# gmh14/tssplat

Measured on AMD Instinct MI355X. Metric: tetrahedra/sec (energy fwd+bwd), higher is better.
Workload: dtype f32

## Files before the change

### tssplat_amd/_build.py

```python
from __future__ import annotations

import contextlib
import hashlib
import os
import shutil
import subprocess
import sys

_HERE = os.path.dirname(os.path.abspath(__file__))
CSRC = os.path.join(_HERE, "csrc")
LIB = os.path.join(_HERE, "libtssplat_amd.so")
_OBJ = os.path.join(_HERE, "_obj")
ARCH = "gfx950"

SOURCES = ["plan.cpp", "plan_mesh.cpp", "plan_tiling.cpp", "plan_layout.cpp", "plan_planes.cpp", "partition.cpp", "conflict_opt.cpp", "regular_batch.cpp", "capi.cpp", "tile_kernel.hip", "step_kernels.hip", "eval_launch.cpp", "surface.cpp", "surface_capi.cpp", "surface_kernels.hip",
           "raster_capi.cpp", "raster_kernels.hip", "aa_kernels.hip", "grid_capi.cpp", "grid_kernels.hip",
           "mlp_capi.cpp", "mlp_kernels.hip", "texture_capi.cpp", "texture_kernels.hip", "shade_capi.cpp", "shade_kernels.hip",
           "init_capi.cpp", "init_kernels.hip", "merge_capi.cpp", "merge_kernels.hip", "fill_kernels.hip",
           "metrics_capi.cpp", "metrics_kernels.hip", "simplify_capi.cpp", "simplify_kernels.hip", "voxel_capi.cpp", "voxel_kernels.hip"]
HEADERS = ["plan.h", "planner.h", "conflict_opt.h", "kernels.h", "launch_args.h", "regular_batch.h", "surface.h", "raster.h", "grid.h", "mlp.h", "texture.h", "shade.h", "init.h", "merge.h", "metrics.h", "simplify.h", "voxel.h", "det_mean.h", "capi_common.h", os.path.join("..", "..", "include", "tssplat_amd.h")]

HOST_FLAGS = ["-O3", "-std=c++17", "-fPIC", "-Wall", "-Wextra", "-Wno-unused-parameter", "-pthread"]
DEVICE_FLAGS = [f"--offload-arch={ARCH}", "-ffp-contract=fast", "-fno-slp-vectorize", "-mllvm", "-amdgpu-sched-strategy=max-ilp"]
SOURCE_FLAGS = {"raster_kernels.hip": ["-ffp-contract=off"], "aa_kernels.hip": ["-ffp-contract=off"],
                "texture_kernels.hip": ["-ffp-contract=off"], "shade_kernels.hip": ["-ffp-contract=off"],
                "init_kernels.hip": ["-ffp-contract=off"], "merge_kernels.hip": ["-ffp-contract=off"],
                "metrics_kernels.hip": ["-ffp-contract=off"], "simplify_kernels.hip": ["-ffp-contract=off"],
                "voxel_kernels.hip": ["-ffp-contract=off"]}


def _hipcc() -> str:
    for cand in (os.environ.get("HIPCC"), shutil.which("hipcc"), "/opt/rocm/bin/hipcc"):
        if cand and os.path.exists(cand):
            return cand
    raise RuntimeError("hipcc not found: the tssplat_amd extension cannot be built (no CPU fallback exists)")


def _digest() -> str:
    h = hashlib.sha256()
    for name in SOURCES + HEADERS:
        with open(os.path.join(CSRC, name), "rb") as fh:
            h.update(fh.read())
    h.update(" ".join(HOST_FLAGS + DEVICE_FLAGS + [f"{k}:{' '.join(v)}" for k, v in sorted(SOURCE_FLAGS.items())]).encode())
    return h.hexdigest()


def traffic_digest() -> str:
    h = hashlib.sha256()
    planner = sorted(n for n in SOURCES + HEADERS if n.startswith("plan") or n.startswith("partition"))
    for name in ["tile_kernel.hip", "launch_args.h"] + planner:
        with open(os.path.join(CSRC, name), "rb") as fh:
            h.update(fh.read())
    return h.hexdigest()[:16]


def build_variant(name: str, extra_device_flags: list[str]) -> str:
    hipcc = _hipcc()
    out = os.path.join(_HERE, f"libtssplat_amd_{name}.so")
    os.makedirs(_OBJ, exist_ok=True)
    objs = []
    for src in SOURCES:
        obj = os.path.join(_OBJ, f"{os.path.splitext(src)[0]}_{name}.o")
        if src.endswith(".hip"):
            cmd = [hipcc, "-c", os.path.join(CSRC, src), "-o", obj] + HOST_FLAGS + DEVICE_FLAGS + SOURCE_FLAGS.get(src, []) + extra_device_flags
        else:
            cmd = [hipcc] + HOST_FLAGS + ["-x", "c++", "-D__HIP_PLATFORM_AMD__", "-I/opt/rocm/include", "-c",
                                           os.path.join(CSRC, src), "-o", obj] + \
                  [f for f in extra_device_flags if f.startswith("-D")]
        subprocess.check_call(cmd)
        objs.append(obj)
    subprocess.check_call([hipcc, "-shared", "-o", out] + objs + [f"--offload-arch={ARCH}", "-pthread"])
    return out


def _write_atomic(path: str, text: str) -> None:
    tmp = f"{path}.{os.getpid()}.tmp"
    with open(tmp, "w") as fh:
        fh.write(text)
    os.replace(tmp, path)


@contextlib.contextmanager
def _build_lock():
    import fcntl
    with open(os.path.join(_HERE, ".build.lock"), "w") as fh:
        fcntl.flock(fh, fcntl.LOCK_EX)
        try:
            yield
        finally:
            fcntl.flock(fh, fcntl.LOCK_UN)


def build(force: bool = False, verbose: bool = False) -> str:
    stamp = LIB + ".digest"
    if not force and os.path.exists(LIB) and os.path.exists(stamp) and open(stamp).read() == _digest():
        return LIB
    with _build_lock():
        return _build_locked(force, verbose)


def _build_locked(force: bool, verbose: bool) -> str:
    stamp = LIB + ".digest"
    digest = _digest()
    if not force and os.path.exists(LIB) and os.path.exists(stamp) and open(stamp).read() == digest:
        return LIB
    hipcc = _hipcc()
    os.makedirs(_OBJ, exist_ok=True)
# ... 69 lines not shown
```

### tssplat_amd/csrc/eval_launch.cpp

```cpp
#include <vector>

#include "kernels.h"
#include "launch_args.h"

namespace tsamd {

bool lane_layout_supported(int spt, int max_threads) { return tile_kernel_for(spt, max_threads, true, false, false, true) != nullptr; }

hipError_t configure_kernels(int lds_bytes)
{
    static int configured[64] = {};
    int dev = 0;
    if (hipGetDevice(&dev) != hipSuccess || dev < 0 || dev >= 64) dev = 0;
    if (lds_bytes <= configured[dev]) return hipSuccess;
    for (const TileKernelRow &row : kTileKernels)
        for (const void *fn : row.fn) {
            hipFuncAttributes attr;
            hipError_t e = hipFuncGetAttributes(&attr, fn);
            if (e != hipSuccess) return e;
            if (attr.sharedSizeBytes != 0) return hipErrorInvalidDeviceFunction;
            e = hipFuncSetAttribute(fn, hipFuncAttributeMaxDynamicSharedMemorySize, lds_bytes);
            if (e != hipSuccess) return e;
        }
    configured[dev] = lds_bytes;
    return hipSuccess;
}

namespace {

struct LaunchRecipe {
    KernelArgs k;
    FinishArgs f;
    const void *tile_fn = nullptr, *finish_fn = nullptr;
    dim3 tile_grid, tile_block, finish_grid, finish_block;
    size_t tile_lds = 0;
};

void set_coefficients(KernelArgs &k, float c1, float c2)
{
    k.c1 = c1;
    k.c2 = c2;
    k.ratio = c2 / c1;
}

hipError_t make_recipe(const EvalArgs &e, LaunchRecipe &r)
{
    if (e.n_tiles > 0) {
        KernelArgs &k = r.k;
        k.tiles = e.tiles;
        k.blob = e.blob;
        k.gvid = e.gvid;
        k.vdst = e.vdst;
        k.x = e.x;
        k.grad_out = e.grad_out;
        k.grad = e.grad;
        k.stage = e.stage;
        k.partials = e.partials;
        set_coefficients(k, e.c1, e.c2);
        k.coef = e.coef;
        k.order = e.order;
        k.n_tiles = int(e.n_tiles);
        k.tiles_per_xcd = int((e.n_tiles + 7) / 8);
        k.vert_stride = e.vert_stride;
        k.n_planes = e.n_planes;
        k.reg_period = uint32_t(e.regular.period);
        k.reg_mul = e.regular.div_mul;
        k.reg_shift = e.regular.div_shift;
        k.reg_v = e.regular.V;
        k.reg_s = e.regular.S;
        r.tile_fn = tile_kernel_for(e.spt, e.block_threads, e.grad != nullptr, e.weighted, e.rebuild, e.index_nt);
        if (!r.tile_fn) return hipErrorInvalidConfiguration;
        r.tile_block = dim3(unsigned(e.block_threads));
        r.tile_grid = dim3(unsigned(8 * k.tiles_per_xcd));
        r.tile_lds = size_t(e.lds_bytes);
    }
    FinishArgs &f = r.f;
    f.fin_vid = e.fin_vid;
    f.fin_off = e.fin_off;
    f.n_finish = e.grad ? e.n_finish : 0;
    f.stage = e.stage;
    f.grad = e.grad;
    f.grad_out = e.grad_out;
    f.partials = e.partials;
    f.n_tiles = e.n_tiles;
    f.c1 = e.c1;
    f.c2 = e.c2;
    f.coef = e.coef;
    f.energy = e.energy;
    f.terms = e.terms;
    f.energy_copy = nullptr;
    const bool regular = e.regular.period > 0 && e.regular.K > 0 && int64_t(finish_grid(e.regular.K) - 1) * 256 >= e.regular.K;
    f.reg_k = regular ? e.regular.K : 0;
    f.reg_copies = regular ? e.regular.copies : 0;
    f.reg_v = regular ? e.regular.V : 0;
    f.reg_s = regular ? e.regular.S : 0;
    if (f.n_finish > 0) {
        r.finish_fn = step_kernels().finish;
        r.finish_grid = regular ? finish_grid_regular(f.reg_k, f.reg_copies) : dim3(finish_grid(f.n_finish));
        r.finish_block = dim3(256);
    } else if (f.energy) {
        r.finish_fn = step_kernels().energy_reduce;
        r.finish_grid = dim3(1);
        r.finish_block = dim3(1024);
    }
    return hipSuccess;
}

hipError_t add_kernel_node(hipGraph_t graph, hipGraphNode_t prev, hipGraphNode_t *node, hipKernelNodeParams &p, const void *fn, dim3 grid, dim3 block,
                           size_t lds, void **args)
{
    p = hipKernelNodeParams{};
    p.func = const_cast<void *>(fn);
    p.gridDim = grid;
    p.blockDim = block;
    p.sharedMemBytes = unsigned(lds);
    p.kernelParams = args;
    p.extra = nullptr;
    return hipGraphAddKernelNode(node, graph, prev ? &prev : nullptr, prev ? 1 : 0, &p);
}

hipError_t launch_eval_kernels(const EvalArgs &e, hipStream_t stream, hipEvent_t *ev)
{
    LaunchRecipe r;
    hipError_t err = make_recipe(e, r);
    if (err != hipSuccess) return err;
    if (r.tile_fn) {
        void *argv[] = {&r.k};
        err = hipLaunchKernel(r.tile_fn, r.tile_grid, r.tile_block, argv, r.tile_lds, stream);
        if (err != hipSuccess) return err;
    }
    if (ev) {
        err = hipEventRecord(ev[1], stream);
        if (err != hipSuccess) return err;
    }
    if (r.finish_fn) {
        void *argv[] = {&r.f};
        err = hipLaunchKernel(r.finish_fn, r.finish_grid, r.finish_block, argv, 0, stream);
        if (err != hipSuccess) return err;
    }
    return hipSuccess;
}

}

hipError_t launch_eval(const EvalArgs &e, hipStream_t stream, hipEvent_t *ev)
{
    if (ev) {
        hipError_t err = hipEventRecord(ev[0], stream);
        if (err != hipSuccess) return err;
    }
    hipError_t rc = launch_eval_kernels(e, stream, ev);
    if (rc == hipSuccess && ev) rc = hipEventRecord(ev[2], stream);
    return rc;
}

struct EvalGraph {
    LaunchRecipe r;
    hipGraph_t graph = nullptr;
    hipGraphExec_t exec = nullptr;
    hipGraphNode_t tile_node = nullptr, finish_node = nullptr;
    hipKernelNodeParams tile_p, finish_p;
    void *tile_argv[1], *finish_argv[1];
    float *own_grad = nullptr;
};

hipError_t eval_graph_create(const EvalArgs &e, EvalGraph **out)
{
    *out = nullptr;
    EvalGraph *g = new EvalGraph();
    hipError_t err = make_recipe(e, g->r);
    g->own_grad = e.grad;
    auto fail = [&](hipError_t code) {
        eval_graph_destroy(g);
        return code;
    };
    if (err != hipSuccess) return fail(err);
    if ((err = hipGraphCreate(&g->graph, 0)) != hipSuccess) return fail(err);
    const LaunchRecipe &r = g->r;
    if (r.tile_fn) {
        g->tile_argv[0] = &g->r.k;
        if ((err = add_kernel_node(g->graph, nullptr, &g->tile_node, g->tile_p, r.tile_fn, r.tile_grid, r.tile_block, r.tile_lds, g->tile_argv)) != hipSuccess)
            return fail(err);
    }
    if (r.finish_fn) {
        g->finish_argv[0] = &g->r.f;
        if ((err = add_kernel_node(g->graph, g->tile_node, &g->finish_node, g->finish_p, r.finish_fn, r.finish_grid, r.finish_block, 0, g->finish_argv)) !=
            hipSuccess)
            return fail(err);
    }
    if ((err = hipGraphInstantiate(&g->exec, g->graph, nullptr, nullptr, 0)) != hipSuccess) return fail(err);
    *out = g;
    return hipSuccess;
}

hipError_t eval_graph_launch(EvalGraph *g, float c1, float c2, hipStream_t stream, float *energy_copy, float *grad)
{
    hipError_t err;
    const bool coef = g->r.k.c1 != c1 || g->r.k.c2 != c2 || g->r.f.c1 != c1 || g->r.f.c2 != c2;
    if (!grad) grad = g->own_grad;
    if (grad != g->r.f.grad && !g->own_grad) return hipErrorInvalidValue;
    const bool moved = grad != g->r.f.grad;
    if (coef || moved) {
        set_coefficients(g->r.k, c1, c2);
        g->r.f.c1 = c1;
        g->r.f.c2 = c2;
        g->r.k.grad = grad;
        if (g->tile_node && (err = hipGraphExecKernelNodeSetParams(g->exec, g->tile_node, &g->tile_p)) != hipSuccess) return err;
    }
    if (coef || moved || g->r.f.energy_copy != energy_copy) {
        if (energy_copy && (!g->finish_node || !g->r.f.energy)) return hipErrorInvalidValue;
        g->r.f.energy_copy = energy_copy;
        g->r.f.grad = grad;
        if (g->finish_node && (err = hipGraphExecKernelNodeSetParams(g->exec, g->finish_node, &g->finish_p)) != hipSuccess) return err;
    }
    return hipGraphLaunch(g->exec, stream);
}

void eval_graph_destroy(EvalGraph *g)
{
    if (!g) return;
    if (g->exec) (void)hipGraphExecDestroy(g->exec);
    if (g->graph) (void)hipGraphDestroy(g->graph);
    delete g;
}

struct TrainLoopGraph {
    struct Adam {
        const float *grad;
        float *g1, *g2, *p;
        int64_t n;
        float b1, b2, lr, bias1, bias2, limit;
        unsigned int *ws;
    };
    struct Step {
        LaunchRecipe r;
        Adam a;
        hipGraphNode_t tile = nullptr, finish = nullptr, moments = nullptr, apply = nullptr;
        hipKernelNodeParams tile_p, finish_p, moments_p, apply_p;
        void *tile_argv[1], *finish_argv[1], *moments_argv[7], *apply_argv[8];
    };
    std::vector<Step> steps;
    hipGraph_t graph = nullptr;
    hipGraphExec_t exec = nullptr;
};

hipError_t train_loop_create(const EvalArgs &e, float *param, float *g1, float *g2, int64_t n_param, void *ws, int n_iters, TrainLoopGraph **out)
{
    *out = nullptr;
    if (n_iters < 1 || n_iters > 4096 || n_param < 1 || !e.grad || !e.energy) return hipErrorInvalidValue;
    TrainLoopGraph *g = new TrainLoopGraph();
    auto fail = [&](hipError_t code) {
        train_loop_destroy(g);
        return code;
    };
    g->steps.resize(size_t(n_iters));
    const StepKernels sk = step_kernels();
    const dim3 adam_blocks(adam_grid(n_param));
    hipError_t err;
    if ((err = hipGraphCreate(&g->graph, 0)) != hipSuccess) return fail(err);
    hipGraphNode_t prev = nullptr;
    {
        hipMemsetParams m = {};
        m.dst = ws;
        m.elementSize = 4;
        m.width = size_t(2 * n_iters);
        m.height = 1;
        m.value = 0;
        if ((err = hipGraphAddMemsetNode(&prev, g->graph, nullptr, 0, &m)) != hipSuccess) return fail(err);
    }
    for (int k = 0; k < n_iters; ++k) {
        TrainLoopGraph::Step &s = g->steps[size_t(k)];
        EvalArgs ek = e;
        ek.x = param;
        ek.energy = e.energy + k;
        if ((err = make_recipe(ek, s.r)) != hipSuccess) return fail(err);
        const LaunchRecipe &r = s.r;
        auto add = [&](hipGraphNode_t *node, hipKernelNodeParams &p, const void *fn, dim3 grid, dim3 block, size_t lds, void **args) {
            const hipError_t rc = add_kernel_node(g->graph, prev, node, p, fn, grid, block, lds, args);
            if (rc == hipSuccess) prev = *node;
            return rc;
        };
        if (r.tile_fn) {
            s.tile_argv[0] = &s.r.k;
            if ((err = add(&s.tile, s.tile_p, r.tile_fn, r.tile_grid, r.tile_block, r.tile_lds, s.tile_argv)) != hipSuccess) return fail(err);
        }
        if (r.finish_fn) {
            s.finish_argv[0] = &s.r.f;
            if ((err = add(&s.finish, s.finish_p, r.finish_fn, r.finish_grid, r.finish_block, 0, s.finish_argv)) != hipSuccess) return fail(err);
        }
        TrainLoopGraph::Adam &a = s.a;
        a = TrainLoopGraph::Adam{e.grad, g1, g2, param, n_param, 0.9f, 0.999f, 0.f, 1.f, 1.f, -1.f, static_cast<unsigned int *>(ws) + 2 * k};
        void **am = s.moments_argv, **aa = s.apply_argv;
        am[0] = &a.grad, am[1] = &a.g1, am[2] = &a.g2, am[3] = &a.n, am[4] = &a.b1, am[5] = &a.b2, am[6] = &a.ws;
        aa[0] = &a.p, aa[1] = &a.g1, aa[2] = &a.n, aa[3] = &a.lr, aa[4] = &a.bias1, aa[5] = &a.bias2, aa[6] = &a.limit, aa[7] = &a.ws;
        if ((err = add(&s.moments, s.moments_p, sk.adam_moments, adam_blocks, dim3(256), 0, am)) != hipSuccess) return fail(err);
        if ((err = add(&s.apply, s.apply_p, sk.adam_apply, adam_blocks, dim3(256), 0, aa)) != hipSuccess) return fail(err);
    }
    if ((err = hipGraphInstantiate(&g->exec, g->graph, nullptr, nullptr, 0)) != hipSuccess) return fail(err);
    *out = g;
    return hipSuccess;
}

hipError_t train_loop_launch(TrainLoopGraph *g, const TrainLoopStep *steps, float lr, float b1, float b2, hipStream_t stream)
{
    hipError_t err;
    for (size_t k = 0; k < g->steps.size(); ++k) {
        TrainLoopGraph::Step &st = g->steps[k];
        LaunchRecipe &r = st.r;
        const TrainLoopStep &s = steps[k];
        if (r.k.c1 != s.c1 || r.k.c2 != s.c2 || r.k.order != s.order || r.f.c1 != s.c1 || r.f.c2 != s.c2) {
            set_coefficients(r.k, s.c1, s.c2);
            r.f.c1 = s.c1;
            r.f.c2 = s.c2;
            r.k.order = s.order;
            if (st.tile && (err = hipGraphExecKernelNodeSetParams(g->exec, st.tile, &st.tile_p)) != hipSuccess) return err;
            if (st.finish && (err = hipGraphExecKernelNodeSetParams(g->exec, st.finish, &st.finish_p)) != hipSuccess) return err;
        }
        TrainLoopGraph::Adam &a = st.a;
        if (a.b1 != b1 || a.b2 != b2) {
            a.b1 = b1;
            a.b2 = b2;
            if ((err = hipGraphExecKernelNodeSetParams(g->exec, st.moments, &st.moments_p)) != hipSuccess) return err;
        }
        if (a.lr != lr || a.bias1 != s.bias1 || a.bias2 != s.bias2 || a.limit != s.limit) {
            a.lr = lr;
            a.bias1 = s.bias1;
            a.bias2 = s.bias2;
            a.limit = s.limit;
            if ((err = hipGraphExecKernelNodeSetParams(g->exec, st.apply, &st.apply_p)) != hipSuccess) return err;
        }
    }
    return hipGraphLaunch(g->exec, stream);
}

void train_loop_destroy(TrainLoopGraph *g)
{
    if (!g) return;
    if (g->exec) (void)hipGraphExecDestroy(g->exec);
    if (g->graph) (void)hipGraphDestroy(g->graph);
    delete g;
}

}
```

### tssplat_amd/csrc/launch_args.h

```cpp
#pragma once

#include <hip/hip_runtime_api.h>

#include <cstdint>

#include "plan.h"

namespace tsamd {

struct KernelArgs {
    const TileDesc *tiles;
    const uint8_t *blob;
    const int32_t *gvid;
    const int32_t *vdst;
    const float *x;
    const float *grad_out;
    float *grad;
    float *stage;
    double *partials;
    float c1, c2;
    float ratio;
    const float *coef;
    int order;
    int n_tiles;
    int tiles_per_xcd;
    int vert_stride;
    int n_planes;
    uint32_t reg_period, reg_mul, reg_shift;
    int reg_v, reg_s;
};

struct FinishArgs {
    const int32_t *fin_vid, *fin_off;
    int64_t n_finish;
    const float *stage;
    float *grad;
    const float *grad_out;
    const double *partials;
    int64_t n_tiles;
    float c1, c2;
    const float *coef;
    float *energy;
    double *terms;
    float *energy_copy;
    int64_t reg_k;
    int reg_copies, reg_v, reg_s;
};

struct TileKernelRow {
    int spt, cap;
    bool weighted, rebuild;
    bool index_nt;
    const void *fn[2];
};
extern const TileKernelRow kTileKernels[9];
const void *tile_kernel_for(int spt, int block_threads, bool grad, bool weighted, bool rebuild, bool index_nt);

struct StepKernels {
    const void *finish, *energy_reduce;
    const void *adam_moments, *adam_apply;
};
StepKernels step_kernels();
unsigned finish_grid(int64_t n_finish);
dim3 finish_grid_regular(int64_t per_copy, int copies);
unsigned adam_grid(int64_t n);

}
```

### tssplat_amd/csrc/tile_kernel.hip

```cpp
#include <hip/hip_runtime.h>

#include "launch_args.h"

namespace tsamd {
namespace {

constexpr int kWave = 64;

#define SLOT_FENCE() __builtin_amdgcn_sched_barrier(0)
#define STAGE_PRIORITY(n) __builtin_amdgcn_s_setprio(n)
#define UNDEF(x) asm volatile("" : "=v"(x))
typedef uint32_t v4u __attribute__((ext_vector_type(4)));
typedef uint32_t v2u __attribute__((ext_vector_type(2)));

__device__ __forceinline__ float det3(const float *F)
{
    return -F[2] * F[4] * F[6] + F[1] * F[5] * F[6] + F[2] * F[3] * F[7] - F[0] * F[5] * F[7] - F[1] * F[3] * F[8] +
           F[0] * F[4] * F[8];
}

__device__ __forceinline__ void cof3(const float *F, float *C)
{
    C[0] = F[4] * F[8] - F[5] * F[7];
    C[1] = F[5] * F[6] - F[3] * F[8];
    C[2] = F[3] * F[7] - F[4] * F[6];
    C[3] = F[2] * F[7] - F[1] * F[8];
    C[4] = F[0] * F[8] - F[2] * F[6];
    C[5] = F[1] * F[6] - F[0] * F[7];
    C[6] = F[1] * F[5] - F[2] * F[4];
    C[7] = F[2] * F[3] - F[0] * F[5];
    C[8] = F[0] * F[4] - F[1] * F[3];
}

#define GLOBAL_AS __attribute__((address_space(1)))
template <class T>
__device__ __forceinline__ GLOBAL_AS T *as_global(T *p)
{
    return (GLOBAL_AS T *)p;
}

typedef float v2f __attribute__((ext_vector_type(2)));
typedef float v4f __attribute__((ext_vector_type(4)));

#define LDS_AS __attribute__((address_space(3)))
template <class T>
__device__ __forceinline__ LDS_AS T *lds_at(uint32_t byte_addr)
{
    return (LDS_AS T *)(uintptr_t)byte_addr;
}

template <class VF>
__device__ __forceinline__ void slot_F(uint32_t xs, uint32_t o0, uint32_t o1, uint32_t o2, uint32_t o3,
                                       const VF *dm, int p, float *F)
{
    const v4u r0 = *lds_at<const v4u>(xs + o0), r1 = *lds_at<const v4u>(xs + o1),
              r2 = *lds_at<const v4u>(xs + o2), r3 = *lds_at<const v4u>(xs + o3);
    asm volatile("" : : "v"(r0), "v"(r1), "v"(r2), "v"(r3));
    const float3 x0 = make_float3(__uint_as_float(r0.x), __uint_as_float(r0.y), __uint_as_float(r0.z));
    const float3 x1 = make_float3(__uint_as_float(r1.x), __uint_as_float(r1.y), __uint_as_float(r1.z));
    const float3 x2 = make_float3(__uint_as_float(r2.x), __uint_as_float(r2.y), __uint_as_float(r2.z));
    const float3 x3 = make_float3(__uint_as_float(r3.x), __uint_as_float(r3.y), __uint_as_float(r3.z));
    const float Ds[9] = {x1.x - x0.x, x2.x - x0.x, x3.x - x0.x, x1.y - x0.y, x2.y - x0.y,
                         x3.y - x0.y, x1.z - x0.z, x2.z - x0.z, x3.z - x0.z};
#pragma unroll
    for (int i = 0; i < 3; ++i)
#pragma unroll
        for (int j = 0; j < 3; ++j)
            F[3 * i + j] = Ds[3 * i + 0] * dm[j][p] + Ds[3 * i + 1] * dm[3 + j][p] + Ds[3 * i + 2] * dm[6 + j][p];
}

template <class VF>
__device__ __forceinline__ void rebuild_dminv(uint32_t rs, uint32_t o0, uint32_t o1, uint32_t o2, uint32_t o3,
                                              VF *dm, int p)
{
    const v4u r0 = *lds_at<const v4u>(rs + o0), r1 = *lds_at<const v4u>(rs + o1),
              r2 = *lds_at<const v4u>(rs + o2), r3 = *lds_at<const v4u>(rs + o3);
    asm volatile("" : : "v"(r0), "v"(r1), "v"(r2), "v"(r3));
    const float x0 = __uint_as_float(r0.x), y0 = __uint_as_float(r0.y), z0 = __uint_as_float(r0.z);
    const float D[9] = {__uint_as_float(r1.x) - x0, __uint_as_float(r2.x) - x0, __uint_as_float(r3.x) - x0,
                        __uint_as_float(r1.y) - y0, __uint_as_float(r2.y) - y0, __uint_as_float(r3.y) - y0,
                        __uint_as_float(r1.z) - z0, __uint_as_float(r2.z) - z0, __uint_as_float(r3.z) - z0};
    float C[9];
    cof3(D, C);
    const float det = D[0] * C[0] + D[1] * C[1] + D[2] * C[2];
    float r = __builtin_amdgcn_rcpf(det);
    r = __builtin_fmaf(__builtin_fmaf(-det, r, 1.f), r, r);
    r = det != 0.f ? r : 0.f;
#pragma unroll
    for (int i = 0; i < 3; ++i)
#pragma unroll
        for (int k = 0; k < 3; ++k) dm[3 * i + k][p] = C[3 * k + i] * r;
}

struct Mat9 {
    v2f p01, p23, p45, p67;
    float p8;
};

__device__ __forceinline__ uint32_t own_token_addr(uint32_t idx) { return 48u * idx + ((idx >> 1) & 12u); }

__device__ __forceinline__ Mat9 load_slot(uint32_t t)
{
    const uint32_t s = t & ~15u;
    const v4f a = *lds_at<const v4f>(s + 16), b = *lds_at<const v4f>(s + 32);
    Mat9 m;
    m.p01 = a.xy; m.p23 = a.zw; m.p45 = b.xy; m.p67 = b.zw;
    m.p8 = *lds_at<const float>(t);
    return m;
}

__device__ __forceinline__ void store_slot(uint32_t t, const float *m)
{
    const uint32_t s = t & ~15u;
    *lds_at<v4f>(s + 16) = v4f{m[0], m[1], m[2], m[3]};
    *lds_at<v4f>(s + 32) = v4f{m[4], m[5], m[6], m[7]};
    *lds_at<float>(t) = m[8];
}

__device__ __forceinline__ void sub9(Mat9 &acc, const Mat9 &g)
{
    acc.p01 -= g.p01; acc.p23 -= g.p23; acc.p45 -= g.p45; acc.p67 -= g.p67;
    acc.p8 -= g.p8;
}

__device__ __forceinline__ Mat9 mat9_of(const float *m)
{
    Mat9 r;
    r.p01 = v2f{m[0], m[1]}; r.p23 = v2f{m[2], m[3]}; r.p45 = v2f{m[4], m[5]}; r.p67 = v2f{m[6], m[7]};
    r.p8 = m[8];
    return r;
}

__device__ __forceinline__ Mat9 laplace_gather(Mat9 acc, const uint32_t *nb)
{
    Mat9 g0 = load_slot(nb[0]);
    acc.p01 *= 4.f; acc.p23 *= 4.f; acc.p45 *= 4.f; acc.p67 *= 4.f;
    acc.p8 *= 4.f;
    Mat9 g1 = load_slot(nb[1]);
    sub9(acc, g0);
    g0 = load_slot(nb[2]);
    sub9(acc, g1);
    g1 = load_slot(nb[3]);
    sub9(acc, g0);
    sub9(acc, g1);
    return acc;
}

__device__ __forceinline__ Mat9 operator_gather(const Mat9 &own, float dg, const float *w, const uint32_t *nb)
{
    Mat9 acc;
    acc.p01 = own.p01 * dg; acc.p23 = own.p23 * dg; acc.p45 = own.p45 * dg; acc.p67 = own.p67 * dg;
    acc.p8 = own.p8 * dg;
#pragma unroll
    for (int k = 0; k < 4; ++k) {
        const Mat9 g = load_slot(nb[k]);
        acc.p01 += g.p01 * w[k]; acc.p23 += g.p23 * w[k]; acc.p45 += g.p45 * w[k]; acc.p67 += g.p67 * w[k];
        acc.p8 += g.p8 * w[k];
    }
    return acc;
}

template <int CTRL>
__device__ __forceinline__ double dpp_f64(double v)
{
    const v2u w = __builtin_bit_cast(v2u, v);
    const v2u r = {uint32_t(__builtin_amdgcn_update_dpp(0, int(w.x), CTRL, 0xf, 0xf, false)),
                   uint32_t(__builtin_amdgcn_update_dpp(0, int(w.y), CTRL, 0xf, 0xf, false))};
    return __builtin_bit_cast(double, r);
}
__device__ __forceinline__ double row_sum_f64(double v)
{
    v += dpp_f64<0xB1>(v);
    v += dpp_f64<0x4E>(v);
    v += dpp_f64<0x124>(v);
    v += dpp_f64<0x128>(v);
    return v;
}

__device__ __forceinline__ float wave_sum(float v)
{
#define TSAMD_DPP(x, ctrl) __builtin_bit_cast(float, __builtin_amdgcn_update_dpp(0, __builtin_bit_cast(int, x), ctrl, 0xf, 0xf, false))
    v += TSAMD_DPP(v, 0xB1);
    v += TSAMD_DPP(v, 0x4E);
    v += TSAMD_DPP(v, 0x124);
    v += TSAMD_DPP(v, 0x128);
#undef TSAMD_DPP
    const int b = __builtin_bit_cast(int, v);
    const float r0 = __builtin_bit_cast(float, __builtin_amdgcn_readlane(b, 0)), r1 = __builtin_bit_cast(float, __builtin_amdgcn_readlane(b, 16)),
                r2 = __builtin_bit_cast(float, __builtin_amdgcn_readlane(b, 32)), r3 = __builtin_bit_cast(float, __builtin_amdgcn_readlane(b, 48));
    return (r0 + r1) + (r2 + r3);
}

constexpr uint32_t kXS = kRowTabBytes;
constexpr uint32_t kZeroEntry = 4u * 66u;

__device__ __forceinline__ uint32_t pos_lo(uint32_t w) { return (w & kVertMask) << 4; }
__device__ __forceinline__ uint32_t pos_hi(uint32_t w) { return ((w >> 16) & kVertMask) << 4; }

template <bool WITH_GRAD, bool WEIGHTED, bool REBUILD, int SPT, bool INDEX_NT>
__device__ __forceinline__ void tile_body(const KernelArgs &a, const int tile, int32_t gv0, const uint32_t reg_vert_off, const int reg_cv, const int reg_cs)
{
    extern __shared__ __attribute__((aligned(16))) unsigned char smem[];
    typedef uint32_t VU __attribute__((ext_vector_type(SPT)));
    typedef float VF __attribute__((ext_vector_type(SPT)));
    static_assert(!(REBUILD && WEIGHTED), "rebuild_dminv is built for the built-in operator");
    constexpr int kKeepF = SPT, kKeepH = WEIGHTED ? 0 : SPT;
    const TileDesc td = a.tiles[tile];
    const int tid = threadIdx.x, nthr = blockDim.x;
    typedef const __attribute__((address_space(4))) float *ConstF;
    const float k_c1 = a.coef ? ((ConstF)(uintptr_t)a.coef)[0] : a.c1, k_c2 = a.coef ? ((ConstF)(uintptr_t)a.coef)[1] : a.c2;
    const float grad_out_scale = WITH_GRAD && a.grad_out ? *(ConstF)(uintptr_t)a.grad_out : 1.f;
    const auto g_blob = as_global(a.blob);
    const auto g_gvid = as_global(a.gvid);
    const auto g_vdst = as_global(a.vdst);
    const auto g_x = as_global(a.x);
    const auto g_grad = as_global(a.grad);
    const auto g_stage = as_global(a.stage);
    const auto g_partials = as_global(a.partials);
    const uint32_t VP = uint32_t(td.n_verts + 3) & ~3u;
    const uint32_t RS = kXS + 16u * VP;
    const uint32_t RB = uint32_t(td.rec_base);
    LDS_AS double *red = lds_at<double>(RB - 256u);
    const int nq = td.s_pad / SPT;
    const bool active = tid < nq;
    const GLOBAL_AS uint32_t *pl = reinterpret_cast<const GLOBAL_AS uint32_t *>(g_blob + td.blob_off);
    const int lt = active ? tid : 0;
    typedef VU PlaneU __attribute__((aligned(SPT == 3 ? 4 : 4 * SPT)));
    typedef VF PlaneF __attribute__((aligned(SPT == 3 ? 4 : 4 * SPT)));
    auto plane_f = [&](int q) -> VF { return __builtin_nontemporal_load(reinterpret_cast<const GLOBAL_AS PlaneF *>(pl + q * td.s_pad + SPT * lt)); };
    constexpr bool kPaired = planes_paired(SPT);
    typedef uint32_t VU2 __attribute__((ext_vector_type(2 * SPT)));
    typedef float VF2 __attribute__((ext_vector_type(2 * SPT)));
    const GLOBAL_AS uint32_t *pli = reinterpret_cast<const GLOBAL_AS uint32_t *>(g_blob + uint64_t(td.stage_off));
#define INDEX_LOAD(p) (INDEX_NT ? __builtin_nontemporal_load(p) : *(p))
    auto pair_u = [&](int q, VU &lo, VU &hi) {
        if (kPaired) {
            const VU2 t = INDEX_LOAD(reinterpret_cast<const GLOBAL_AS VU2 *>(pli + q * td.s_pad + 2 * SPT * lt));
#pragma unroll
            for (int p = 0; p < SPT; ++p) lo[p] = t[p], hi[p] = t[SPT + p];
        } else {
            lo = INDEX_LOAD(reinterpret_cast<const GLOBAL_AS PlaneU *>(pli + q * td.s_pad + SPT * lt));
            hi = INDEX_LOAD(reinterpret_cast<const GLOBAL_AS PlaneU *>(pli + (q + 1) * td.s_pad + SPT * lt));
        }
    };
    auto pair_f = [&](int q, VF &lo, VF &hi) {
        if (kPaired) {
            const VF2 t = __builtin_nontemporal_load(reinterpret_cast<const GLOBAL_AS VF2 *>(pl + q * td.s_pad + 2 * SPT * lt));
#pragma unroll
            for (int p = 0; p < SPT; ++p) lo[p] = t[p], hi[p] = t[SPT + p];
        } else {
            lo = plane_f(q), hi = plane_f(q + 1);
        }
    };
    asm volatile("" : "+v"(gv0));
    float px, py, pz;
    {
        const size_t gv = size_t(gv0 + reg_cv) * 3;
        px = g_x[gv], py = g_x[gv + 1], pz = g_x[gv + 2];
    }
    __builtin_amdgcn_sched_barrier(0);
    VU q_lv01, q_lv23, q_nb01, q_nb23;
    pair_u(0, q_lv01, q_lv23);
    VF dm[9];
    const int kBasePlanes = REBUILD ? kPlanesRebuild : (WEIGHTED ? a.n_planes : kPlanes);
    const GLOBAL_AS uint16_t *g_rowtab = reinterpret_cast<const GLOBAL_AS uint16_t *>(pli + size_t(kBasePlanes) * td.s_pad);
    const GLOBAL_AS v4f *g_rest = reinterpret_cast<const GLOBAL_AS v4f *>(reinterpret_cast<const GLOBAL_AS uint16_t *>(pl + size_t(kBasePlanes) * td.s_pad) + kRowTabEntries);
    v4f rest0 = v4f{0.f, 0.f, 0.f, 0.f};
    if (REBUILD) rest0 = g_rest[tid < td.n_verts ? tid : 0];
    __builtin_amdgcn_sched_barrier(0);
    if (!REBUILD) {
#pragma unroll
        for (int c = 0; c < 8; c += 2) pair_f(4 + c, dm[c], dm[c + 1]);
        dm[8] = plane_f(12);
    }
    __builtin_amdgcn_sched_barrier(0);
    if (tid < td.n_verts) {
        *lds_at<v4f>(kXS + 16u * uint32_t(tid)) = v4f{px, py, pz, 0.f};
        if (REBUILD) *lds_at<v4f>(RS + 16u * uint32_t(tid)) = rest0;
    }
    for (int v = tid + nthr; v < td.n_verts; v += nthr) {
        const size_t gv = size_t(g_gvid[td.vert_off + v]) * 3;
        *lds_at<v4f>(kXS + 16u * uint32_t(v)) = v4f{g_x[gv], g_x[gv + 1], g_x[gv + 2], 0.f};
        if (REBUILD) *lds_at<v4f>(RS + 16u * uint32_t(v)) = g_rest[v];
    }
    __syncthreads();
    pair_u(2, q_nb01, q_nb23);
    VF wd, wk[4];
    if (WEIGHTED) {
        wd = plane_f(13);
        pair_f(14, wk[0], wk[1]);
        pair_f(16, wk[2], wk[3]);
    }
    uint32_t row0 = 0;
    if (WITH_GRAD) row0 = INDEX_LOAD(&g_rowtab[tid < 65 ? tid : 64]);
    __builtin_amdgcn_sched_barrier(0);

    const float ratio = a.coef ? k_c2 / k_c1 : a.ratio;
    const bool factored = k_c1 != 0.f && __builtin_fabsf(ratio) <= 0x1p+40f;
    const float s_pen = factored ? ratio : k_c2, out_scale = factored ? k_c1 : 1.f, q_scale = factored ? 1.f : k_c1;
    uint32_t t_own_reg[SPT];
#pragma unroll
    for (int p = 0; p < SPT; ++p) t_own_reg[p] = RB + own_token_addr(uint32_t(p * nq + tid));
    auto t_own_at = [&](int p) -> uint32_t {
        if (!WEIGHTED) return t_own_reg[p];
        uint32_t t = uint32_t(tid);
        asm volatile("" : "+v"(t));
        return RB + own_token_addr(uint32_t(p * nq) + t);
    };
#define t_own(p) t_own_at(p)
    auto is_owned = [&](int p) { return p * nq + tid < td.n_owned; };

    STAGE_PRIORITY(0);
    float scal[SPT];
#pragma unroll
    for (int p = 0; p < SPT; ++p) scal[p] = 0.f;
    float e_b = 0.f, e_s = 0.f;
    float Fk[kKeepF > 0 ? kKeepF : 1][9];
#pragma unroll
    for (int p = 0; p < kKeepF; ++p)
#pragma unroll
        for (int c = 0; c < 9; ++c) UNDEF(Fk[p][c]);
    if (active) {
#pragma unroll
        for (int p = 0; p < SPT; ++p) {
            const uint32_t w0 = q_lv01[p], w1 = q_lv23[p];
            if (REBUILD) rebuild_dminv(RS, pos_lo(w0), pos_hi(w0), pos_lo(w1), pos_hi(w1), dm, p);
            float F[9];
            slot_F(kXS, pos_lo(w0), pos_hi(w0), pos_lo(w1), pos_hi(w1), dm, p, F);
            if (p < kKeepF) {
#pragma unroll
                for (int c = 0; c < 9; ++c) Fk[p][c] = F[c];
            }
            if (is_owned(p)) {
                const float J = det3(F);
                const float Jm = fmaxf(-J, 0.f);
                float pen = 0.f, dpen = 0.f;
                if (a.order == 2) {
                    pen = Jm * Jm;
                    dpen = -2.f * Jm;
                } else if (a.order == 4) {
                    pen = Jm * Jm * Jm * Jm;
                    dpen = -4.f * Jm * Jm * Jm;
                }
// ... 132 lines not shown
            for (int p = 0; p < SPT; ++p)
#pragma unroll
                for (int c = 0; c < 9; ++c) UNDEF(D[p][c]);
        }
        uint32_t fdst[SPT][4];
#pragma unroll
        for (int p = 0; p < SPT; ++p) {
            const uint32_t w0 = q_lv01[p], w1 = q_lv23[p];
            const uint32_t r0 = *lds_at<const uint32_t>((w0 >> 8) & 0xfcu), r1 = *lds_at<const uint32_t>((w0 >> 24) & 0xfcu),
                           r2 = *lds_at<const uint32_t>((w1 >> 8) & 0xfcu), r3 = *lds_at<const uint32_t>((w1 >> 24) & 0xfcu);
            fdst[p][0] = (w0 & kVertMask) * 12u + r0;
            fdst[p][1] = ((w0 >> 16) & kVertMask) * 12u + r1;
            fdst[p][2] = (w1 & kVertMask) * 12u + r2;
            fdst[p][3] = ((w1 >> 16) & kVertMask) * 12u + r3;
        }
        int vb0 = wave;
        if (wave & 4) {
            const int g4 = wave & ~3, top = g4 + 3 < nw - 1 ? g4 + 3 : nw - 1;
            vb0 = g4 + (top - wave);
        }
        int32_t dst_row = 0;
        if (64 * vb0 + lane < td.n_verts) dst_row = INDEX_LOAD(&g_vdst[reg_vert_off + uint32_t(64 * vb0 + lane)]);
        __syncthreads();
        STAGE_PRIORITY(3);
        if (active) {
#pragma unroll
            for (int p = 0; p < SPT; ++p) {
                if (p * nq + tid < td.n_slots) {
                    const float *d = D[p];
                    LDS_AS float *f0 = lds_at<float>(fdst[p][0]), *f1 = lds_at<float>(fdst[p][1]), *f2 = lds_at<float>(fdst[p][2]),
                                 *f3 = lds_at<float>(fdst[p][3]);
                    f0[0] = (-d[0] - d[3]) - d[6], f0[1] = (-d[1] - d[4]) - d[7], f0[2] = (-d[2] - d[5]) - d[8];
                    f1[0] = d[0], f1[1] = d[1], f1[2] = d[2];
                    f2[0] = d[3], f2[1] = d[4], f2[2] = d[5];
                    f3[0] = d[6], f3[1] = d[7], f3[2] = d[8];
                }
            }
        }
        __syncthreads();

        const float gscale = grad_out_scale * out_scale;
        const uint32_t tab = *lds_at<const uint32_t>(4u * uint32_t(lane));
        const uint32_t wid = *lds_at<const uint32_t>(4u * uint32_t(lane) + 4u) - tab;
        auto vertex_sums = [&](int vb, int32_t row, int cv, int cs) {
            const int v = 64 * vb + lane;
            const uint32_t v12 = 12u * uint32_t(v);
            const int rows = __builtin_popcountll(__builtin_amdgcn_ballot_w64(wid > 768u * uint32_t(vb)));
            float gx = 0.f, gy = 0.f, gz = 0.f;
            for (int r = 0; r < rows; r += 4) {
                const LDS_AS float *f[4];
#pragma unroll
                for (int u = 0; u < 4; ++u) {
                    const uint32_t base = uint32_t(__builtin_amdgcn_readlane(int(tab), r + u)), w = uint32_t(__builtin_amdgcn_readlane(int(wid), r + u));
                    f[u] = lds_at<const float>(v12 < w ? base + v12 : kZeroEntry);
                }
#pragma unroll
                for (int u = 0; u < 4; ++u) {
                    gx += f[u][0];
                    gy += f[u][1];
                    gz += f[u][2];
                }
            }
            if (v < td.n_verts) {
                const bool excl = row >= 0;
                GLOBAL_AS float *dst = (excl ? g_grad : g_stage) + size_t(excl ? row + cv : ~row + cs) * 3;
                const float sc = excl ? gscale : out_scale;
                dst[0] = gx * sc;
                dst[1] = gy * sc;
                dst[2] = gz * sc;
            }
        };
        if (64 * vb0 < td.n_verts) vertex_sums(vb0, dst_row, reg_cv, reg_cs);
        if (64 * nw < td.n_verts) {
            for (int vb = vb0 + nw; 64 * vb < td.n_verts; vb += nw)
                vertex_sums(vb, 64 * vb + lane < td.n_verts ? g_vdst[td.vert_off + 64 * vb + lane] : 0, 0, 0);
        }
        sum_waves();
    }
#undef t_own
#undef INDEX_LOAD
}

template <bool WITH_GRAD, bool WEIGHTED, bool REBUILD, int SPT, bool INDEX_NT>
__device__ __forceinline__ void tile_entry(const KernelArgs &a)
{
    const int xcd = blockIdx.x & 7, jb = blockIdx.x >> 3;
    const int tile_end = (xcd + 1) * a.tiles_per_xcd < a.n_tiles ? (xcd + 1) * a.tiles_per_xcd : a.n_tiles;
    const int tile = xcd * a.tiles_per_xcd + jb;
    if (jb >= a.tiles_per_xcd || tile >= tile_end) return;
    const uint32_t reg_c = uint32_t((uint64_t(uint32_t(tile)) * a.reg_mul) >> a.reg_shift);
    const uint32_t reg_r = uint32_t(tile) - reg_c * a.reg_period;
    const uint32_t reg_vert_off = reg_r * uint32_t(a.vert_stride);
    const GLOBAL_AS int32_t *gv_ptr = &as_global(a.gvid)[size_t(reg_r) * size_t(a.vert_stride) + size_t(int(threadIdx.x) < a.vert_stride ? threadIdx.x : 0)];
    const int32_t gv0 = INDEX_NT ? __builtin_nontemporal_load(gv_ptr) : *gv_ptr;
    __builtin_amdgcn_sched_barrier(0);
    tile_body<WITH_GRAD, WEIGHTED, REBUILD, SPT, INDEX_NT>(a, tile, gv0, reg_vert_off, int(reg_c) * a.reg_v, int(reg_c) * a.reg_s);
}

template <bool WITH_GRAD, int BLOCK, int WPE, bool WEIGHTED = false, bool REBUILD = false, int SPT = kSlotsPerLane>
__global__ __launch_bounds__(BLOCK, WPE) void tile_energy_kernel(const KernelArgs a)
{
    tile_entry<WITH_GRAD, WEIGHTED, REBUILD, SPT, true>(a);
}

template <bool WITH_GRAD, int BLOCK, int WPE, bool WEIGHTED = false, bool REBUILD = false>
__global__ __launch_bounds__(BLOCK, WPE) void tile_shared_index_kernel(const KernelArgs a)
{
    tile_entry<WITH_GRAD, WEIGHTED, REBUILD, kSlotsPerLane, false>(a);
}

}

#define TSAMD_FN(...) {reinterpret_cast<const void *>(&tile_energy_kernel<false, __VA_ARGS__>), reinterpret_cast<const void *>(&tile_energy_kernel<true, __VA_ARGS__>)}
#define TSAMD_FN_SHARED(...) {reinterpret_cast<const void *>(&tile_shared_index_kernel<false, __VA_ARGS__>), reinterpret_cast<const void *>(&tile_shared_index_kernel<true, __VA_ARGS__>)}
const TileKernelRow kTileKernels[9] = {
    {2, 768, true, false, false, TSAMD_FN_SHARED(768, 6, true, false)},
    {2, 768, false, true, false, TSAMD_FN_SHARED(768, 6, false, true)},
    {2, 768, false, false, false, TSAMD_FN_SHARED(768, 6, false, false)},
    {2, 768, true, false, true, TSAMD_FN(768, 6, true, false, 2)},
    {2, 768, false, true, true, TSAMD_FN(768, 6, false, true, 2)},
    {2, 768, false, false, true, TSAMD_FN(768, 6, false, false, 2)},
    {3, 512, false, false, true, TSAMD_FN(512, 4, false, false, 3)},
    {4, 768, false, false, true, TSAMD_FN(768, 3, false, false, 4)},
    {3, 1024, false, false, true, TSAMD_FN(1024, 4, false, false, 3)},
};
#undef TSAMD_FN
#undef TSAMD_FN_SHARED

const void *tile_kernel_for(int spt, int block_threads, bool grad, bool weighted, bool rebuild, bool index_nt)
{
    rebuild = rebuild && !weighted;
    for (const TileKernelRow &row : kTileKernels)
        if (row.spt == spt && block_threads <= row.cap && row.weighted == weighted && row.rebuild == rebuild && (row.index_nt || !index_nt))
            return row.fn[grad];
    return nullptr;
}

}
```

Baseline: 65.71 billion.

## Preload tile kernel head arguments into SGPRs and prefetch the tile descriptor early

Splits the tile kernel's argument struct into 14 dwords of scalar head parameters (tile count, division constants, stride, and the gvid/tiles/x/blob pointers), passed as separate kernel arguments and preloaded into SGPRs with the kernarg-preload compiler flag. The descriptor is loaded in the entry function as three quads, and the vertex position load moves ahead of the coefficient loads. The coefficient and grad_out loads become unconditional scalar loads that fall back to a dummy address. The aim is to shorten each block's startup latency from kernarg memory loads. In exchange it adds a fragile ABI coupling through the static_assert on the 14-dword window, and touches every launch path.

```diff
diff --git a/tssplat_amd/_build.py b/tssplat_amd/_build.py
--- a/tssplat_amd/_build.py
+++ b/tssplat_amd/_build.py
@@ -22,7 +22,8 @@
 
 HOST_FLAGS = ["-O3", "-std=c++17", "-fPIC", "-Wall", "-Wextra", "-Wno-unused-parameter", "-pthread"]
 DEVICE_FLAGS = [f"--offload-arch={ARCH}", "-ffp-contract=fast", "-fno-slp-vectorize", "-mllvm", "-amdgpu-sched-strategy=max-ilp"]
-SOURCE_FLAGS = {"raster_kernels.hip": ["-ffp-contract=off"], "aa_kernels.hip": ["-ffp-contract=off"],
+SOURCE_FLAGS = {"tile_kernel.hip": ["-mllvm", "-amdgpu-kernarg-preload-count=16"],
+                "raster_kernels.hip": ["-ffp-contract=off"], "aa_kernels.hip": ["-ffp-contract=off"],
                 "texture_kernels.hip": ["-ffp-contract=off"], "shade_kernels.hip": ["-ffp-contract=off"],
                 "init_kernels.hip": ["-ffp-contract=off"], "merge_kernels.hip": ["-ffp-contract=off"],
                 "metrics_kernels.hip": ["-ffp-contract=off"], "simplify_kernels.hip": ["-ffp-contract=off"],
diff --git a/tssplat_amd/csrc/eval_launch.cpp b/tssplat_amd/csrc/eval_launch.cpp
--- a/tssplat_amd/csrc/eval_launch.cpp
+++ b/tssplat_amd/csrc/eval_launch.cpp
@@ -29,6 +29,7 @@
 namespace {
 
 struct LaunchRecipe {
+    TileHeadArgs h;
     KernelArgs k;
     FinishArgs f;
     const void *tile_fn = nullptr, *finish_fn = nullptr;
@@ -46,12 +47,13 @@
 hipError_t make_recipe(const EvalArgs &e, LaunchRecipe &r)
 {
     if (e.n_tiles > 0) {
+        TileHeadArgs &h = r.h;
         KernelArgs &k = r.k;
-        k.tiles = e.tiles;
-        k.blob = e.blob;
-        k.gvid = e.gvid;
+        h.tiles = e.tiles;
+        h.blob = e.blob;
+        h.gvid = e.gvid;
         k.vdst = e.vdst;
-        k.x = e.x;
+        h.x = e.x;
         k.grad_out = e.grad_out;
         k.grad = e.grad;
         k.stage = e.stage;
@@ -59,19 +61,18 @@
         set_coefficients(k, e.c1, e.c2);
         k.coef = e.coef;
         k.order = e.order;
-        k.n_tiles = int(e.n_tiles);
-        k.tiles_per_xcd = int((e.n_tiles + 7) / 8);
-        k.vert_stride = e.vert_stride;
+        h.n_tiles = int(e.n_tiles);
+        h.vert_stride = e.vert_stride;
         k.n_planes = e.n_planes;
-        k.reg_period = uint32_t(e.regular.period);
-        k.reg_mul = e.regular.div_mul;
-        k.reg_shift = e.regular.div_shift;
-        k.reg_v = e.regular.V;
+        h.reg_period = uint32_t(e.regular.period);
+        h.reg_mul = e.regular.div_mul;
+        h.reg_shift = e.regular.div_shift;
+        h.reg_v = e.regular.V;
         k.reg_s = e.regular.S;
         r.tile_fn = tile_kernel_for(e.spt, e.block_threads, e.grad != nullptr, e.weighted, e.rebuild, e.index_nt);
         if (!r.tile_fn) return hipErrorInvalidConfiguration;
         r.tile_block = dim3(unsigned(e.block_threads));
-        r.tile_grid = dim3(unsigned(8 * k.tiles_per_xcd));
+        r.tile_grid = dim3(unsigned(8 * tiles_per_xcd(h.n_tiles)));
         r.tile_lds = size_t(e.lds_bytes);
     }
     FinishArgs &f = r.f;
@@ -125,7 +126,8 @@
     hipError_t err = make_recipe(e, r);
     if (err != hipSuccess) return err;
     if (r.tile_fn) {
-        void *argv[] = {&r.k};
+        void *argv[kTileKernelParams];
+        tile_kernel_params(r.h, r.k, argv);
         err = hipLaunchKernel(r.tile_fn, r.tile_grid, r.tile_block, argv, r.tile_lds, stream);
         if (err != hipSuccess) return err;
     }
@@ -160,7 +162,7 @@
     hipGraphExec_t exec = nullptr;
     hipGraphNode_t tile_node = nullptr, finish_node = nullptr;
     hipKernelNodeParams tile_p, finish_p;
-    void *tile_argv[1], *finish_argv[1];
+    void *tile_argv[kTileKernelParams], *finish_argv[1];
     float *own_grad = nullptr;
 };
 
@@ -178,7 +180,7 @@
     if ((err = hipGraphCreate(&g->graph, 0)) != hipSuccess) return fail(err);
     const LaunchRecipe &r = g->r;
     if (r.tile_fn) {
-        g->tile_argv[0] = &g->r.k;
+        tile_kernel_params(g->r.h, g->r.k, g->tile_argv);
         if ((err = add_kernel_node(g->graph, nullptr, &g->tile_node, g->tile_p, r.tile_fn, r.tile_grid, r.tile_block, r.tile_lds, g->tile_argv)) != hipSuccess)
             return fail(err);
     }
@@ -237,7 +239,7 @@
         Adam a;
         hipGraphNode_t tile = nullptr, finish = nullptr, moments = nullptr, apply = nullptr;
         hipKernelNodeParams tile_p, finish_p, moments_p, apply_p;
-        void *tile_argv[1], *finish_argv[1], *moments_argv[7], *apply_argv[8];
+        void *tile_argv[kTileKernelParams], *finish_argv[1], *moments_argv[7], *apply_argv[8];
     };
     std::vector<Step> steps;
     hipGraph_t graph = nullptr;
@@ -281,7 +283,7 @@
             return rc;
         };
         if (r.tile_fn) {
-            s.tile_argv[0] = &s.r.k;
+            tile_kernel_params(s.r.h, s.r.k, s.tile_argv);
             if ((err = add(&s.tile, s.tile_p, r.tile_fn, r.tile_grid, r.tile_block, r.tile_lds, s.tile_argv)) != hipSuccess) return fail(err);
         }
         if (r.finish_fn) {
diff --git a/tssplat_amd/csrc/launch_args.h b/tssplat_amd/csrc/launch_args.h
--- a/tssplat_amd/csrc/launch_args.h
+++ b/tssplat_amd/csrc/launch_args.h
@@ -8,12 +8,34 @@
 
 namespace tsamd {
 
+#define TSAMD_TILE_HEAD_FIELDS(X)                                                                                                              \
+    X(int, n_tiles)                                                                                                                            \
+        \
+             \
+                                                                         \
+    X(uint32_t, reg_mul)                                                                                                                       \
+    X(uint32_t, reg_shift)                                                                                                                     \
+    X(uint32_t, reg_period)                                                                                                                    \
+    X(int, reg_v)                                                                                                                              \
+    X(int, vert_stride)         \
+    X(const int32_t *, gvid)                                                                                                                 \
+    X(const TileDesc *, tiles)                                                                                                                 \
+    X(const float *, x)                                                                                                                        \
+    X(const uint8_t *, blob)
+
+struct TileHeadArgs {
+#define TSAMD_X(type, name) type name;
+    TSAMD_TILE_HEAD_FIELDS(TSAMD_X)
+#undef TSAMD_X
+};
+#define TSAMD_X(type, name) +1
+constexpr int kTileHeadParams = 0 TSAMD_TILE_HEAD_FIELDS(TSAMD_X);
+#undef TSAMD_X
+constexpr int kTileKernelParams = kTileHeadParams + 1;
+static_assert(sizeof(TileHeadArgs) == 14 * 4, "the head arguments are sized for the 14-dword preload window, without padding");
+
 struct KernelArgs {
-    const TileDesc *tiles;
-    const uint8_t *blob;
-    const int32_t *gvid;
     const int32_t *vdst;
-    const float *x;
     const float *grad_out;
     float *grad;
     float *stage;
@@ -22,13 +44,20 @@
     float ratio;
     const float *coef;
     int order;
-    int n_tiles;
-    int tiles_per_xcd;
-    int vert_stride;
     int n_planes;
-    uint32_t reg_period, reg_mul, reg_shift;
-    int reg_v, reg_s;
+    int reg_s;
 };
+
+constexpr int tiles_per_xcd(int n_tiles) { return (n_tiles + 7) >> 3; }
+
+inline void tile_kernel_params(TileHeadArgs &h, KernelArgs &k, void *(&argv)[kTileKernelParams])
+{
+    int n = 0;
+#define TSAMD_X(type, name) argv[n++] = &h.name;
+    TSAMD_TILE_HEAD_FIELDS(TSAMD_X)
+#undef TSAMD_X
+    argv[n] = &k;
+}
 
 struct FinishArgs {
     const int32_t *fin_vid, *fin_off;
diff --git a/tssplat_amd/csrc/tile_kernel.hip b/tssplat_amd/csrc/tile_kernel.hip
--- a/tssplat_amd/csrc/tile_kernel.hip
+++ b/tssplat_amd/csrc/tile_kernel.hip
@@ -41,6 +41,11 @@
 
 typedef float v2f __attribute__((ext_vector_type(2)));
 typedef float v4f __attribute__((ext_vector_type(4)));
+
+struct TileDescWords {
+    v4u q0, q1, q2;
+};
+static_assert(sizeof(TileDescWords) == sizeof(TileDesc), "a tile descriptor is three quads");
 
 #define LDS_AS __attribute__((address_space(3)))
 template <class T>
@@ -198,22 +203,35 @@
 __device__ __forceinline__ uint32_t pos_hi(uint32_t w) { return ((w >> 16) & kVertMask) << 4; }
 
 template <bool WITH_GRAD, bool WEIGHTED, bool REBUILD, int SPT, bool INDEX_NT>
-__device__ __forceinline__ void tile_body(const KernelArgs &a, const int tile, int32_t gv0, const uint32_t reg_vert_off, const int reg_cv, const int reg_cs)
+__device__ __forceinline__ void tile_body(const TileHeadArgs &h, const KernelArgs &a, const int tile, int32_t gv0, TileDescWords tdw, const uint32_t reg_vert_off, const int reg_cv,
+                                          const int reg_cs)
 {
     extern __shared__ __attribute__((aligned(16))) unsigned char smem[];
     typedef uint32_t VU __attribute__((ext_vector_type(SPT)));
     typedef float VF __attribute__((ext_vector_type(SPT)));
     static_assert(!(REBUILD && WEIGHTED), "rebuild_dminv is built for the built-in operator");
     constexpr int kKeepF = SPT, kKeepH = WEIGHTED ? 0 : SPT;
-    const TileDesc td = a.tiles[tile];
     const int tid = threadIdx.x, nthr = blockDim.x;
+    const auto g_blob = as_global(h.blob);
+    const auto g_gvid = as_global(h.gvid);
+    const auto g_vdst = as_global(a.vdst);
+    const auto g_x = as_global(h.x);
+    asm volatile("" : "+v"(gv0));
+    float px, py, pz;
+    {
+        const size_t gv = size_t(gv0 + reg_cv) * 3;
+        px = g_x[gv], py = g_x[gv + 1], pz = g_x[gv + 2];
+    }
+    __builtin_amdgcn_sched_barrier(0);
+    asm volatile("" : "+s"(tdw.q0), "+s"(tdw.q1), "+s"(tdw.q2));
+    const TileDesc td = __builtin_bit_cast(TileDesc, tdw);
     typedef const __attribute__((address_space(4))) float *ConstF;
-    const float k_c1 = a.coef ? ((ConstF)(uintptr_t)a.coef)[0] : a.c1, k_c2 = a.coef ? ((ConstF)(uintptr_t)a.coef)[1] : a.c2;
-    const float grad_out_scale = WITH_GRAD && a.grad_out ? *(ConstF)(uintptr_t)a.grad_out : 1.f;
-    const auto g_blob = as_global(a.blob);
-    const auto g_gvid = as_global(a.gvid);
-    const auto g_vdst = as_global(a.vdst);
-    const auto g_x = as_global(a.x);
+    typedef v2f CoefPair __attribute__((aligned(4)));
+    typedef const __attribute__((address_space(4))) CoefPair *ConstF2;
+    const v2f dev_coef = *(ConstF2)(uintptr_t)(a.coef ? (const void *)a.coef : (const void *)h.tiles);
+    const float dev_grad_out = *(ConstF)(uintptr_t)(WITH_GRAD && a.grad_out ? (const void *)a.grad_out : (const void *)h.tiles);
+    const float k_c1 = a.coef ? dev_coef.x : a.c1, k_c2 = a.coef ? dev_coef.y : a.c2;
+    const float grad_out_scale = WITH_GRAD && a.grad_out ? dev_grad_out : 1.f;
     const auto g_grad = as_global(a.grad);
     const auto g_stage = as_global(a.stage);
     const auto g_partials = as_global(a.partials);
@@ -252,13 +270,6 @@
             lo = plane_f(q), hi = plane_f(q + 1);
         }
     };
-    asm volatile("" : "+v"(gv0));
-    float px, py, pz;
-    {
-        const size_t gv = size_t(gv0 + reg_cv) * 3;
-        px = g_x[gv], py = g_x[gv + 1], pz = g_x[gv + 2];
-    }
-    __builtin_amdgcn_sched_barrier(0);
     VU q_lv01, q_lv23, q_nb01, q_nb23;
     pair_u(0, q_lv01, q_lv23);
     VF dm[9];
@@ -557,32 +568,40 @@
 }
 
 template <bool WITH_GRAD, bool WEIGHTED, bool REBUILD, int SPT, bool INDEX_NT>
-__device__ __forceinline__ void tile_entry(const KernelArgs &a)
+__device__ __forceinline__ void tile_entry(const TileHeadArgs &h, const KernelArgs &a)
 {
     const int xcd = blockIdx.x & 7, jb = blockIdx.x >> 3;
-    const int tile_end = (xcd + 1) * a.tiles_per_xcd < a.n_tiles ? (xcd + 1) * a.tiles_per_xcd : a.n_tiles;
-    const int tile = xcd * a.tiles_per_xcd + jb;
-    if (jb >= a.tiles_per_xcd || tile >= tile_end) return;
-    const uint32_t reg_c = uint32_t((uint64_t(uint32_t(tile)) * a.reg_mul) >> a.reg_shift);
-    const uint32_t reg_r = uint32_t(tile) - reg_c * a.reg_period;
-    const uint32_t reg_vert_off = reg_r * uint32_t(a.vert_stride);
-    const GLOBAL_AS int32_t *gv_ptr = &as_global(a.gvid)[size_t(reg_r) * size_t(a.vert_stride) + size_t(int(threadIdx.x) < a.vert_stride ? threadIdx.x : 0)];
+    const int per_xcd = tiles_per_xcd(h.n_tiles);
+    const int tile_end = (xcd + 1) * per_xcd < h.n_tiles ? (xcd + 1) * per_xcd : h.n_tiles;
+    const int tile = xcd * per_xcd + jb;
+    if (jb >= per_xcd || tile >= tile_end) return;
+    typedef const __attribute__((address_space(4))) v4u *ConstQuad;
+    const ConstQuad td_ptr = (ConstQuad)(uintptr_t)(h.tiles + tile);
+    const TileDescWords tdw = {td_ptr[0], td_ptr[1], td_ptr[2]};
+    const uint32_t reg_c = uint32_t((uint64_t(uint32_t(tile)) * h.reg_mul) >> h.reg_shift);
+    const uint32_t reg_r = uint32_t(tile) - reg_c * h.reg_period;
+    const uint32_t reg_vert_off = reg_r * uint32_t(h.vert_stride);
+    const GLOBAL_AS int32_t *gv_ptr = &as_global(h.gvid)[size_t(reg_r) * size_t(h.vert_stride) + size_t(int(threadIdx.x) < h.vert_stride ? threadIdx.x : 0)];
     const int32_t gv0 = INDEX_NT ? __builtin_nontemporal_load(gv_ptr) : *gv_ptr;
     __builtin_amdgcn_sched_barrier(0);
-    tile_body<WITH_GRAD, WEIGHTED, REBUILD, SPT, INDEX_NT>(a, tile, gv0, reg_vert_off, int(reg_c) * a.reg_v, int(reg_c) * a.reg_s);
-}
-
+    tile_body<WITH_GRAD, WEIGHTED, REBUILD, SPT, INDEX_NT>(h, a, tile, gv0, tdw, reg_vert_off, int(reg_c) * h.reg_v, int(reg_c) * a.reg_s);
+}
+
+#define TSAMD_HEAD_PARAM(type, name) type const name,
+#define TSAMD_HEAD_VALUE(type, name) name,
 template <bool WITH_GRAD, int BLOCK, int WPE, bool WEIGHTED = false, bool REBUILD = false, int SPT = kSlotsPerLane>
-__global__ __launch_bounds__(BLOCK, WPE) void tile_energy_kernel(const KernelArgs a)
-{
-    tile_entry<WITH_GRAD, WEIGHTED, REBUILD, SPT, true>(a);
+__global__ __launch_bounds__(BLOCK, WPE) void tile_energy_kernel(TSAMD_TILE_HEAD_FIELDS(TSAMD_HEAD_PARAM) const KernelArgs a)
+{
+    tile_entry<WITH_GRAD, WEIGHTED, REBUILD, SPT, true>(TileHeadArgs{TSAMD_TILE_HEAD_FIELDS(TSAMD_HEAD_VALUE)}, a);
 }
 
 template <bool WITH_GRAD, int BLOCK, int WPE, bool WEIGHTED = false, bool REBUILD = false>
-__global__ __launch_bounds__(BLOCK, WPE) void tile_shared_index_kernel(const KernelArgs a)
-{
-    tile_entry<WITH_GRAD, WEIGHTED, REBUILD, kSlotsPerLane, false>(a);
-}
+__global__ __launch_bounds__(BLOCK, WPE) void tile_shared_index_kernel(TSAMD_TILE_HEAD_FIELDS(TSAMD_HEAD_PARAM) const KernelArgs a)
+{
+    tile_entry<WITH_GRAD, WEIGHTED, REBUILD, kSlotsPerLane, false>(TileHeadArgs{TSAMD_TILE_HEAD_FIELDS(TSAMD_HEAD_VALUE)}, a);
+}
+#undef TSAMD_HEAD_PARAM
+#undef TSAMD_HEAD_VALUE
 
 }
 
```

New measurement: 65.78 billion (median of 4 runs). No clear change (+0.1%).
